# srtee/lammps-USER-CONP2

Measured on AMD Instinct MI355X. Metric: charge-solve updates/sec + ns/day, 4096-atom electrode / 32k electrolyte, higher is better.
Workload: dtype f64; 1 GPU; synthetic graphene/IL 4096 electrode + 32768 electrolyte, ffield; Ne=4096, Nl=32768, K=99773, kflat=645, mode=ffield, solver=inv, kspace=ewald, blist_pairs=302717, structure_factor_form=z-window (32 columns, grid 480)

## Files before the change

### include/conp_hip.h

```cpp
#ifndef CONP_HIP_H
#define CONP_HIP_H

#include <stddef.h>
#include <stdint.h>

#ifdef __cplusplus
extern "C" {
#endif

#define CONP_ABI_VERSION 1

typedef enum {
  CONP_OK = 0,
  CONP_ERR_ARG = -1,
  CONP_ERR_STATE = -2,
  CONP_ERR_NO_DEVICE = -3,
  CONP_ERR_NUMERIC = -4,
  CONP_ERR_IO = -5
} conp_status;

enum { CONP_FF_NORMAL = 0, CONP_FF_FFIELD = 1, CONP_FF_NOSLAB = 2 };
enum { CONP_SOLVER_CG = 0, CONP_SOLVER_INV = 1 };

typedef struct conp_fix conp_fix;
// ... 114 lines not shown
                              double *energy ,
                              double *virial ,
                              double *eatom  );

int conp_pppm_compute_forces(conp_fix *fix, const conp_atoms *atoms,
                             double *f      ,
                             double *energy ,
                             double *virial ,
                             double *eatom  );

typedef struct {
  int pairflag, kspaceflag, qsumflag;
  double eta;
} conp_potential_args;
int conp_compute_potential_atom(conp_fix *fix, const conp_atoms *atoms, const conp_neighlist *pairlist, const int *sel,
                                const int *etasel , const conp_potential_args *args, double *potential);

typedef struct {
  int elenum, elenum_all, elytenum, maxtag_all, runstage;
  int kcount, kcount_flat, kcount_expand, kxmax, kymax, kzmax, kmax, kmax3d;
  int kcount_dims[7];
  int cg_iterations;
  int n_zclasses;
  double unitk[3], volume, gsqmx, ug_tot, totsetq, scalar_output, totinve, slabcorr;
  int64_t n_blist_pairs, n_alist_pairs, n_elyte_charged;
  int inverse_path;
  int inverse_retries;
  int pppm_elyte_spreads;
  int zn_cols, zn_grid, zn_rows;
  int zn_ranges;
  int hc_arithmetic;
  int zc_final;
  int zc_row_tiles;
} conp_info;
int conp_fix_info(const conp_fix *fix, conp_info *out);
int conp_fix_get_ktables(const conp_fix *fix, int *kxvecs, int *kyvecs, int *kzvecs, double *ug, int *kxy_list, int *kz_list);
int conp_fix_get_maps(const conp_fix *fix, int *ele2tag, int *ele2eleall, int *eleall2tag, int *eleall2ele,
                      int *elecheck_eleall, int *elebuf2eleall, int *tag2eleall);
int conp_fix_get_matrix(conp_fix *fix, double *aaa_all );
int conp_fix_set_matrix(conp_fix *fix, const double *aaa_all, int runstage);
int conp_fix_get_vectors(conp_fix *fix, double *bbb_all, double *eleallq, double *elesetq);
int conp_fix_get_sfac(conp_fix *fix, double *sfacrl, double *sfacim);
int conp_fix_get_ele_trig(conp_fix *fix, double *csk, double *snk);
int conp_inv_project(conp_fix *fix, int n, double *aaa, int nullneutral, int zneutr, const double *eleallz, double zhalf,
                     double *totinve_out);

int conp_fix_write_matrix_file(conp_fix *fix, const char *path, int which);
int conp_fix_read_matrix_file(conp_fix *fix, const conp_atoms *atoms, const char *path);

int conp_invert(conp_fix *fix, int n, double *aaa);

int conp_host_ktables(double g_ewald, double accuracy, double slab_volfactor, int slabflag, double xprd, double yprd, double zprd,
                      double qsqsum, int64_t natoms, double qqrd2e, double dielectric, int *info , int *kxvecs,
                      int *kyvecs, int *kzvecs, double *ug, int *kxy_list, int *kz_list, int *plan_p, int *plan_m, int *plan_sign);
int conp_host_index(int n0, const int *tag0, const int *echeck0, int n1, const int *tag1, const int *echeck1, int *sizes,
                    int *ele2tag, int *ele2eleall, int *eleall2tag, int *eleall2ele, int *elebuf2eleall, int *tag2eleall);
int64_t conp_host_pair_rows(int which, const conp_neighlist *list, const conp_atoms *atoms, int newton, int *row_ptr,
                            int *ele_atom, int *oth_atom, int *col);

int conp_fix_set_stream(conp_fix *fix, void *hip_stream);
int conp_fix_bind_device_buffers(conp_fix *fix, double *d_b , double *d_q );
int conp_fix_row_range(const conp_fix *fix, int *row0, int *row1);
int conp_fix_b_cal_device(conp_fix *fix, const double *d_x, const double *d_q);
int conp_fix_solve_device(conp_fix *fix, double potdiff);
int conp_fix_scatter_device(conp_fix *fix, double *d_q_atoms, double potdiff);
int conp_fix_pre_force_device(conp_fix *fix, const double *d_x, double *d_q, double potdiff);
// ... 35 lines not shown
  int nlocal, nall;
  double cutneigh;
  const int *d_tag, *d_nspecial, *d_special;
  int maxspecial;
  double prd_half[3];
} conp_pair_build_args;
int conp_pair_build_list_device(conp_fix *fix, const double *d_x, const conp_pair_build_args *a);
int conp_pair_list_moved_device(conp_fix *fix, const double *d_x, double trigger, int *d_flag);
int conp_pair_get_list(conp_fix *fix, int *inum, int *nall, int64_t *nneigh,
                       int *ilist, int *numneigh, int *first, int *neigh);

int conp_fix_profile(conp_fix *fix, int enable);
int conp_fix_profile_read(conp_fix *fix, int *nkernels, const char **names , double *avg_ms , int *counts );
int conp_fix_pin_host_arrays(conp_fix *fix, const double *x, const double *q, int n);
int conp_fix_unpin_host_arrays(conp_fix *fix);
void *conp_host_alloc(size_t bytes);
void conp_host_free(void *p);

int conp_debug_check_guards(void);

enum {
  CONP_PATH_PARTIAL_TILES = 1 << 0,
  CONP_PATH_A_GENERAL = 1 << 1,
  CONP_PATH_INV_PIVOTED = 1 << 2,
  CONP_PATH_CG_TWO_LAUNCH = 1 << 3,
  CONP_PATH_GEMV_ROWS = 1 << 4,
  CONP_PATH_PHASE_LAUNCH = 1 << 5,
  CONP_PATH_PPPM_SPREAD_LAUNCH = 1 << 6,
  CONP_PATH_ROWS_HOST = 1 << 7,
  CONP_PATH_TIME_SPLIT = 1 << 8,
  CONP_PATH_SK_CLASSIC = 1 << 12,
  CONP_PATH_ZN_WIDE = 1 << 13,
  CONP_PATH_ZC_PHASE_LOADS = 1 << 14,
  CONP_PATH_HC_TABLES = 1 << 15
};
void conp_debug_set_paths(unsigned mask);
void conp_debug_set_sk_workgroups(int n);
void conp_debug_set_ew_block(int n);


int conp_fix_write_timing(conp_fix *fix);
const char *conp_fix_log_drain(conp_fix *fix);
const char *conp_fix_mesg_drain(conp_fix *fix);

#ifdef __cplusplus
}
#endif
#endif
```

### lammps-user-conp2_amd/conp_amd/capi.py

```python
from __future__ import annotations

import ctypes as C
import os
from typing import Optional, Sequence

import numpy as np

from . import systems as _systems

HERE = os.path.dirname(os.path.abspath(__file__))
_LIB = None


class ConpError(RuntimeError):
    def __init__(self, code, msg):
        super().__init__(f"[conp status {code}] {msg}")
        self.code = code
        self.msg = msg


def library_path():
    return os.environ.get("CONP_LIB") or os.path.join(HERE, "libconp_hip.so")


# ... 32 lines not shown
_CB_GATHERV = C.CFUNCTYPE(C.c_int, C.c_void_p, C.c_void_p, C.c_int64, C.c_void_p, C.POINTER(C.c_int64), C.POINTER(C.c_int64))


class conp_comm(C.Structure):
    _fields_ = [("ctx", C.c_void_p), ("rank", C.c_int), ("nranks", C.c_int), ("allreduce_sum", _CB_SUM),
                ("allreduce_max_int", _CB_MAXI), ("allgather_int", _CB_GATHER_INT), ("allgatherv", _CB_GATHERV)]


class conp_potential_args(C.Structure):
    _fields_ = [("pairflag", C.c_int), ("kspaceflag", C.c_int), ("qsumflag", C.c_int), ("eta", C.c_double)]


class conp_pair_params(C.Structure):
    _fields_ = [("ntypes", C.c_int), ("cutsq", C.POINTER(C.c_double)), ("cut_coul", C.c_double),
                ("cut_ljsq", C.POINTER(C.c_double)), ("lj1", C.POINTER(C.c_double)), ("lj2", C.POINTER(C.c_double)),
                ("lj3", C.POINTER(C.c_double)), ("lj4", C.POINTER(C.c_double)), ("offset", C.POINTER(C.c_double)),
                ("special_lj", C.c_double * 4), ("special_coul", C.c_double * 4)]


class conp_pair_build_args(C.Structure):
    _fields_ = [("nlocal", C.c_int), ("nall", C.c_int), ("cutneigh", C.c_double), ("d_tag", C.c_void_p), ("d_nspecial", C.c_void_p),
                ("d_special", C.c_void_p), ("maxspecial", C.c_int), ("prd_half", C.c_double * 3)]


class conp_info(C.Structure):
    _fields_ = [("elenum", C.c_int), ("elenum_all", C.c_int), ("elytenum", C.c_int), ("maxtag_all", C.c_int),
                ("runstage", C.c_int), ("kcount", C.c_int), ("kcount_flat", C.c_int), ("kcount_expand", C.c_int),
                ("kxmax", C.c_int), ("kymax", C.c_int), ("kzmax", C.c_int), ("kmax", C.c_int), ("kmax3d", C.c_int),
                ("kcount_dims", C.c_int * 7), ("cg_iterations", C.c_int), ("n_zclasses", C.c_int), ("unitk", C.c_double * 3),
                ("volume", C.c_double), ("gsqmx", C.c_double), ("ug_tot", C.c_double), ("totsetq", C.c_double),
                ("scalar_output", C.c_double), ("totinve", C.c_double), ("slabcorr", C.c_double),
                ("n_blist_pairs", C.c_int64), ("n_alist_pairs", C.c_int64), ("n_elyte_charged", C.c_int64),
                ("inverse_path", C.c_int), ("inverse_retries", C.c_int), ("pppm_elyte_spreads", C.c_int), ("zn_cols", C.c_int), ("zn_grid", C.c_int), ("zn_rows", C.c_int),
                ("zn_ranges", C.c_int), ("hc_arithmetic", C.c_int), ("zc_final", C.c_int), ("zc_row_tiles", C.c_int)]


SYMBOLS = [
    "conp_parse_fix_args", "conp_fix_create", "conp_fix_destroy", "conp_last_error", "conp_abi_version",
    "conp_fix_init_list", "conp_fix_setup_post_neighbor", "conp_fix_setup_pre_force", "conp_fix_post_neighbor",
    "conp_fix_pre_force", "conp_fix_compute_scalar", "conp_fix_post_force", "conp_fix_post_force_step", "conp_fix_modify_param", "conp_fix_linalg_setup", "conp_fix_a_cal", "conp_fix_b_cal",
    "conp_fix_equation_solve", "conp_fix_update_charge", "conp_km_conp_setup", "conp_km_a_cal", "conp_km_b_cal",
    "conp_fix_info", "conp_fix_get_ktables", "conp_fix_get_maps", "conp_fix_get_matrix", "conp_fix_set_matrix",
    "conp_fix_get_vectors", "conp_fix_get_sfac", "conp_fix_get_ele_trig", "conp_inv_project", "conp_invert",
    "conp_host_ktables", "conp_host_index", "conp_host_pair_rows", "conp_fix_write_matrix_file", "conp_fix_read_matrix_file",
    "conp_fix_set_stream",
    "conp_fix_bind_device_buffers", "conp_fix_row_range", "conp_fix_b_cal_device", "conp_fix_solve_device",
    "conp_fix_scatter_device", "conp_fix_pre_force_device", "conp_fix_profile", "conp_fix_profile_read", "conp_debug_check_guards",
    "conp_debug_set_paths", "conp_debug_set_sk_workgroups", "conp_debug_set_ew_block",
    "conp_fix_pin_host_arrays", "conp_fix_unpin_host_arrays", "conp_host_alloc", "conp_host_free",
    "conp_fix_write_timing", "conp_fix_log_drain", "conp_fix_mesg_drain",
    "conp_fix_set_comm", "conp_rccl_unique_id", "conp_fix_comm_init_rccl", "conp_rccl_available", "conp_fix_comm_destroy_rccl",
    "conp_pppm_make_rho", "conp_pppm_compute_group_potential", "conp_pppm_compute_particle_potential",
    "conp_pppm_keep_density", "conp_pppm_compute",
    "conp_ewald_compute", "conp_ewald_compute_group_potential", "conp_ewald_compute_particle_potential",
    "conp_ewald_compute_forces", "conp_pppm_compute_forces",
    "conp_ewald_compute_forces_device", "conp_pppm_compute_forces_device",
    "conp_ewald_compute_forces_vatom", "conp_pppm_compute_forces_vatom",
    "conp_ewald_compute_forces_vatom_device", "conp_pppm_compute_forces_vatom_device",
    "conp_compute_potential_atom",
    "conp_pair_set_params", "conp_pair_set_list", "conp_pair_compute", "conp_pair_compute_device",
    "conp_pair_build_list_device", "conp_pair_list_moved_device", "conp_pair_get_list",
]


PATH_PARTIAL_TILES, PATH_A_GENERAL, PATH_INV_PIVOTED, PATH_CG_TWO_LAUNCH, PATH_GEMV_ROWS = 1, 2, 4, 8, 16
PATH_PHASE_LAUNCH, PATH_PPPM_SPREAD_LAUNCH, PATH_ROWS_HOST, PATH_TIME_SPLIT = 32, 64, 128, 256
PATH_SK_CLASSIC = 4096
PATH_ZN_WIDE = 8192
PATH_ZC_PHASE_LOADS = 16384
PATH_HC_TABLES = 32768


class test_paths:

    def __init__(self, mask=0, sk_workgroups=0):
        self.mask, self.nwg = mask, sk_workgroups

    def __enter__(self):
        lib = load_library()
        if not hasattr(lib, "conp_debug_set_paths"):
            raise RuntimeError("this library build has no test hooks (a comparison build of an earlier round?)")
        lib.conp_debug_set_paths(self.mask)
        lib.conp_debug_set_sk_workgroups(self.nwg)
        return self

    def __exit__(self, *a):
        lib = load_library()
        lib.conp_debug_set_paths(0)
        lib.conp_debug_set_sk_workgroups(0)
        return False


def set_ew_block(n: int):
    load_library().conp_debug_set_ew_block(int(n))


def load_library():
    global _LIB
    if _LIB is not None:
        return _LIB
    path = library_path()
    if not os.path.exists(path):
        raise ImportError(f"{path} is missing: build it with `python -c 'import __graft_entry__ as g; g.build()'` "
# ... 672 lines not shown
```

### lammps-user-conp2_amd/csrc/conp_fix.cpp

```cpp
#include <hip/hip_runtime.h>
#include <dlfcn.h>
#include <rccl/rccl.h>

#include <algorithm>
#include <cmath>
#include <cstdarg>
#include <chrono>
#include <cstdio>
#include <cstdlib>
#include <cstring>
#include <map>
#include <memory>
#include <mutex>
#include <stdexcept>
#include <string>
#include <vector>

#include "../../include/conp_hip.h"
#include "conp_host.hpp"
#include "conp_kernels.h"

namespace {

thread_local std::string g_last_error;
// ... 278 lines not shown
  double cond_vmult = 0.0;
  bool cond_ready = false;
  std::vector<int> elyte_idx_h;
  int bl_inum = 0;
  size_t bl_nneigh = 0;
  DevBuf<char> d_rows_scratch;
  int nlocal_cur = 0;
  hipStream_t stream = nullptr;
  bool own_stream = false;
  DevBuf<double> d_x, d_q, d_qc, d_slab_part, d_Gpart, d_G, d_Gw, d_wfull, d_Rp, d_Tz, d_ele_z, d_bk, d_breal, d_b_own,
      d_eleallq_own, d_qele, d_elesetq, d_eleinitq, d_A, d_cutsq, d_scalars, d_ainve, d_sfr, d_sfi, d_cg_res, d_cg_p, d_Srows, d_xg, d_qg, d_pp_ele, d_pp_scratch,
      d_cg_ap, d_cg_scal, d_inv_work, d_inv_backup, d_Tzc, d_TzcT, d_Hpart, d_Hc, d_Wz, d_Spk, d_yp, d_f, d_pfacc, d_pp_coeff, d_pp_green, d_pp_tw0, d_pp_tw1,
      d_pp_tw2, d_pp_re, d_pp_im, d_pp_ew, d_eta_ij, d_fo_ij, d_u0_i, d_diag_atom, d_setzvec;
  DevBuf<double2> d_Xt, d_Yt, d_Zt, d_Xe, d_Ye;
  DevBuf<int> d_type, d_atom2eleall, d_elyte_idx, d_p_ikx, d_p_iky, d_p_sgn, d_sf_row_a, d_sf_col_c, d_k_sign, d_k_p, d_k_m,
      d_elecheck, d_zclass, d_nb_act, d_rt_mine, d_own_rt, d_own_pv, d_ele_pairs, d_a_chunk_group, d_ct_ptr, d_seg_ptr, d_seg_idx, d_hslot_ptr, d_hslot_idx, d_b_rowptr, d_b_ele, d_b_oth, d_a_rowptr, d_a_ele, d_a_oth, d_a_col, d_bl_ilist, d_bl_numneigh, d_bl_first, d_bl_neigh, d_pp_egrid, d_ipiv, d_info, d_cg_done, d_iota, d_ele_csr_ptr, d_ele_csr_of, d_ele_csr_row;
  bool left_stale = false;
  double left_potdiff = 0.0;
  DevBuf<unsigned char> d_mask;
  DevBuf<SkItem> d_items;
  DevBuf<SkWItem> d_witems;
  int witems_maxseg = 1;
  DevBuf<SkProj> d_skproj;
  SkProj skproj_h{};
  DevBuf<SkFuse> d_skfuse;
  SkFuse skfuse_h{};
  DevBuf<SkTile> d_tiles;
  double *d_b = nullptr, *d_eleallq = nullptr;
  bool b_bound = false, q_bound = false;
  int n_slab_part = 0;
  const bool sk_partials = path_on(CONP_PATH_PARTIAL_TILES);
  const bool time_split = path_on(CONP_PATH_TIME_SPLIT);
  const bool gemv_rows = path_on(CONP_PATH_GEMV_ROWS);
  const bool no_phase_fuse = path_on(CONP_PATH_PHASE_LAUNCH);
  int table_c0 = 0, table_c1 = 0;
  int hslots = 0;
  bool g_current = true;
  int max_nsplit = 0;
  int n_slots = 0;
  DevPlan dplan{};
  Profiler prof;

  ~conp_fix() {
    if (time_host && th[5] > 0)
      std::fprintf(stderr, "conp host-buffer update, us per call over %.0f calls: list check %.1f, staging + H2D enqueue %.1f, kernel "
                           "enqueue %.1f, solve enqueue + wait + D2H %.1f, scatter %.1f\n", th[5], 1e6 * th[0] / th[5], 1e6 * th[1] / th[5],
                   1e6 * th[2] / th[5], 1e6 * th[3] / th[5], 1e6 * th[4] / th[5]);
    prof.collect();
    drop_graph();
    if (nccl) { (void)hipStreamSynchronize(stream); (void)g_rccl.CommDestroy(nccl); nccl = nullptr; }
    if (pin_x || pin_q) { (void)hipStreamSynchronize(stream); if (pin_x) (void)hipHostUnregister(const_cast<double *>(pin_x)); if (pin_q) (void)hipHostUnregister(const_cast<double *>(pin_q)); }
    if (h_pin) { (void)hipStreamSynchronize(stream); (void)hipHostFree(h_pin); }
    if (h_np) { (void)hipStreamSynchronize(stream); (void)hipHostFree(h_np); }
    if (ren_arena) { (void)hipStreamSynchronize(stream); (void)hipHostFree(ren_arena); ren_arena = nullptr; }
    if (zn_flag_host) { (void)hipStreamSynchronize(stream); (void)hipHostFree(zn_flag_host); zn_flag_host = nullptr; }
    for (auto &e : ev_b) if (e) (void)hipEventDestroy(e);
    if (own_stream && stream) (void)hipStreamDestroy(stream);
  }

  RealParams real_params() const {
    RealParams rp;
    rp.g_ewald = env.g_ewald; rp.eta = args.eta;
    double cut_coulsq = env.cut_coul * env.cut_coul;
    const double cut_erfc = 5.8 * 5.8 / (env.g_ewald * env.g_ewald);
    if (cut_coulsq > cut_erfc) cut_coulsq = cut_erfc;
    rp.cut_coulsq = cut_coulsq; rp.ntypes = env.ntypes; rp.cutsq = d_cutsq.p;
// ... 1680 lines not shown
                                           "two collectives yourself between conp_fix_b_cal_device / _solve_device / _scatter_device)");
    prof.end(stream);
  }
  void allgather_q() {
    if ((env.nranks <= 1 && !nccl) || args.minimizer != CONP_SOLVER_INV) return;
    const int ne = idx.elenum_all;
    prof.begin("allgather_q", stream);
    if (nccl) {
      double *mine = d_eleallq + (size_t)env.rank * rows_per;
      g_rccl.ok(g_rccl.AllGather(mine, d_eleallq, (size_t)rows_per, ncclDouble, nccl, stream), "all-gather(q)");
    } else if (rc.active()) {
      double *h = pinned((size_t)ne_pad + 8 + (size_t)ne + rows_per) + ne_pad + 8;
      const int nr = row1 - row0;
      if (nr) HIP_TRY(hipMemcpyAsync(h + ne, d_eleallq + row0, nr * sizeof(double), hipMemcpyDeviceToHost, stream));
      sync();
      std::vector<int> rows(env.nranks);
      for (int r = 0; r < env.nranks; ++r) rows[r] = std::min(ne, (r + 1) * rows_per) - std::min(ne, r * rows_per);
      rc.gatherv(h + ne, rows, 1, h);
      HIP_TRY(hipMemcpyAsync(d_eleallq, h, ne * sizeof(double), hipMemcpyHostToDevice, stream));
    }
    prof.end(stream);
  }

  bool can_fuse_solve() const {
    return args.minimizer == CONP_SOLVER_INV && !args.conq && !args.cond && env.nranks == 1 && !nccl && !s_sharded &&
           runstage >= 3;
  }
  long s_generation = 0, spk_of = -1;
  bool spk_symmetric = false;
  DevBuf<unsigned long long> d_symstat;
  bool use_sym_gemv() const {
    return !gemv_rows && idx.elenum_all >= 2048;
  }
  void solve_scatter_fused(double *d_q_atoms, double potdiff) {
    const int ne = idx.elenum_all;
    if (use_sym_gemv()) {
      if (spk_of != s_generation) {
        d_Spk.reserve(sym_packed_doubles(ne_pad));
        d_yp.reserve((size_t)(ne_pad / 128) * ne_pad);
        d_symstat.reserve(2);
        launch_sym_pack(stream, ne, ne_pad, d_A.p, d_Spk.p, d_symstat.p);
        unsigned long long st[2] = {0, 0};
        HIP_TRY(hipMemcpyAsync(st, d_symstat.p, sizeof st, hipMemcpyDeviceToHost, stream));
        sync();
        double mx, md;
        std::memcpy(&mx, &st[0], sizeof mx); std::memcpy(&md, &st[1], sizeof md);
        spk_symmetric = md <= 1e-10 * mx;
        spk_of = s_generation;
        if (!spk_symmetric)
          mesgf("conp/hip: the solve matrix is not symmetric (max |S_ij - S_ji| = %.3g, max |S_ij| = %.3g): full rows are multiplied\n", md, mx);
      }
    }
    if (use_sym_gemv() && spk_symmetric) {
      prof.begin("gemv_charge", stream);
      launch_sym_gemv_finish(stream, ne, ne_pad, d_Spk.p, d_b, d_yp.p, d_eleallq, d_elesetq.p, args.qinit ? d_eleinitq.p : nullptr,
                             potdiff, d_ele_csr_ptr.p, d_ele_csr_of.p, d_ele_csr_row.p, d_qele.p, d_q_atoms);
      prof.end(stream);
      left_stale = true; left_potdiff = potdiff;
      HIP_TRY(hipGetLastError());
      return;
    }
    prof.begin("gemv_charge", stream);
    launch_gemv_finish(stream, ne, d_A.p, d_b, d_eleallq, d_elesetq.p, args.qinit ? d_eleinitq.p : nullptr, potdiff, d_ele_csr_ptr.p,
                       d_ele_csr_of.p, d_qele.p, d_q_atoms);
    prof.end(stream);
    left_stale = true; left_potdiff = potdiff;
    HIP_TRY(hipGetLastError());
  }

  void scatter_device(double *d_q_atoms, double potdiff, bool labelled = true) {
    const int ne = idx.elenum_all;
    if (labelled) prof.begin("charge_write", stream);
    if (args.cond) {
      if (!cond_ready) {
        std::vector<double> sq(ne), sz(ne);
        HIP_TRY(hipMemcpyAsync(sq.data(), d_elesetq.p, ne * sizeof(double), hipMemcpyDeviceToHost, stream));
        HIP_TRY(hipMemcpyAsync(sz.data(), d_setzvec.p, ne * sizeof(double), hipMemcpyDeviceToHost, stream));
        sync();
        double zOAz = 0.;
        for (int i = 0; i < ne; ++i) zOAz += sq[i] * sz[i];
        double vm = 4 * 3.14159265358979323846 * zOAz * env.zprd / (evscale * env.xprd * env.yprd);
        vm /= 1 + vm;
        vm /= zOAz;
        cond_vmult = vm;
        cond_ready = true;
      }
      launch_cond_potdiff(stream, ne, d_setzvec.p, d_eleallq, d_slab_part.p, n_slab_part, env.zprd, potdiff, cond_vmult,
                          d_scalars.p + 3);
      launch_charge_finish(stream, ne, n_ele_atoms, d_ele_pairs.p, d_elecheck.p, d_eleallq, d_elesetq.p,
                           args.qinit ? d_eleinitq.p : nullptr, 0.0, d_scalars.p + 3, d_qele.p, d_q_atoms, nullptr);
    } else if (args.conq) {
      launch_left_sum(stream, ne, d_elecheck.p, d_eleallq, d_scalars.p + 1);
      launch_conq_potdiff(stream, d_scalars.p + 1, potdiff, totsetq, env.one_electrode, d_scalars.p + 3);
      launch_charge_finish(stream, ne, n_ele_atoms, d_ele_pairs.p, d_elecheck.p, d_eleallq, d_elesetq.p,
// ... 676 lines not shown
  if (!f->tables_current) f->km_a_read(at);
  if (at->nlocal + at->nghost != f->nall) throw ConpError(CONP_ERR_STATE, "atom count changed without post_neighbor");
  if (f->elyte_list_stale(at)) { f->sync(); f->build_elyte_list(at); }
  f->upload_xq(at);
  if (f->decomposed) f->gather_elyte(at);
  f->b_cal_device(f->d_x.p, f->d_q.p, false);
  if (f->nccl || f->rc.active()) f->allreduce_b();
  HIP_TRY(hipMemcpyAsync(bbb, f->d_b, f->idx.elenum_all * sizeof(double), hipMemcpyDeviceToHost, f->stream));
  f->sync();
  CONP_GUARD_END
}

int conp_fix_info(const conp_fix *f, conp_info *o) {
  CONP_GUARD_BEGIN
  std::memset(o, 0, sizeof(*o));
  o->elenum = f->idx.elenum; o->elenum_all = f->idx.elenum_all; o->elytenum = f->idx.elytenum;
  o->maxtag_all = f->idx.maxtag_all; o->runstage = f->runstage;
  o->kcount = f->kt.kcount; o->kcount_flat = f->kt.kcount_flat; o->kcount_expand = f->kt.kcount_expand;
  o->kxmax = f->kt.kxmax; o->kymax = f->kt.kymax; o->kzmax = f->kt.kzmax; o->kmax = f->kt.kmax; o->kmax3d = f->kt.kmax3d;
  for (int i = 0; i < 7; ++i) o->kcount_dims[i] = f->kt.kcount_dims[i];
  o->cg_iterations = f->cg_iterations;
  o->n_zclasses = f->nzc;
  for (int i = 0; i < 3; ++i) o->unitk[i] = f->kt.unitk[i];
  o->volume = f->kt.volume; o->gsqmx = f->kt.gsqmx; o->ug_tot = f->kt.ug_tot; o->totsetq = f->totsetq;
  o->scalar_output = f->scalar_output; o->totinve = f->totinve; o->slabcorr = f->slabcorr;
  int64_t nbp = f->n_b_pairs;
  if (f->np_pending) { HIP_TRY(hipStreamSynchronize(f->stream)); nbp = *f->h_np; }
  o->n_blist_pairs = nbp;
  o->inverse_path = f->inverse_path; o->inverse_retries = f->inverse_retries; o->pppm_elyte_spreads = f->pp_elyte_spreads;
  const bool zn_on = f->zn_use() || f->zn_gen_use();
  o->zn_cols = zn_on ? 16 * f->zn_ncf : 0; o->zn_grid = zn_on ? f->zn_n : 0; o->zn_rows = zn_on ? 128 * (int)f->own_rt_h.size() : 0; o->n_alist_pairs = f->arows.npairs(); o->n_elyte_charged = f->nl;
  o->zn_ranges = zn_on ? f->zn_nrg : 0; o->hc_arithmetic = f->zn_use() && f->zn_frag_arith ? 1 : 0;
  o->zc_final = f->zc_final_form; o->zc_row_tiles = f->zc_final_form ? (int)f->own_rt_h.size() : 0;
  CONP_GUARD_END
}

int conp_fix_get_ktables(const conp_fix *f, int *kx, int *ky, int *kz, double *ug, int *kxy_list, int *kz_list) {
  CONP_GUARD_BEGIN
  if (!f->kspace_ready) throw ConpError(CONP_ERR_STATE, "k tables not built");
  const size_t K = f->kt.kcount, E = f->kt.kcount_expand;
  if (kx) std::memcpy(kx, f->kt.kxvecs.data(), K * sizeof(int));
  if (ky) std::memcpy(ky, f->kt.kyvecs.data(), K * sizeof(int));
  if (kz) std::memcpy(kz, f->kt.kzvecs.data(), K * sizeof(int));
  if (ug) std::memcpy(ug, f->kt.ug.data(), K * sizeof(double));
  if (kxy_list) std::memcpy(kxy_list, f->kt.kxy_list.data(), E * sizeof(int));
  if (kz_list) std::memcpy(kz_list, f->kt.kz_list.data(), E * sizeof(int));
  CONP_GUARD_END
}

int conp_fix_get_maps(const conp_fix *f, int *ele2tag, int *ele2eleall, int *eleall2tag, int *eleall2ele,
                      int *elecheck_eleall, int *elebuf2eleall, int *tag2eleall) {
  CONP_GUARD_BEGIN
  const EleIndex &x = f->idx;
  auto cp = [](int *dst, const std::vector<int> &v) { if (dst && !v.empty()) std::memcpy(dst, v.data(), v.size() * sizeof(int)); };
  cp(ele2tag, x.ele2tag); cp(ele2eleall, x.ele2eleall); cp(eleall2tag, x.eleall2tag); cp(eleall2ele, x.eleall2ele);
  cp(elecheck_eleall, x.elecheck_eleall); cp(elebuf2eleall, x.elebuf2eleall); cp(tag2eleall, x.tag2eleall);
  CONP_GUARD_END
}

int conp_fix_get_matrix(conp_fix *f, double *aaa) {
  CONP_GUARD_BEGIN
  f->drop_graph();
  f->unshard_rows();
  const size_t ne = f->idx.elenum_all;
  HIP_TRY(hipMemcpyAsync(aaa, f->d_A.p, ne * ne * sizeof(double), hipMemcpyDeviceToHost, f->stream));
  f->sync();
// ... 1216 lines not shown
```

### lammps-user-conp2_amd/csrc/conp_kernels.h

```cpp
#pragma once
#include <hip/hip_runtime.h>
#include <atomic>
#include <cstddef>
#include <cstdint>
#include "../../include/conp_hip.h"

namespace conp {

bool path_on(unsigned bit);
int debug_sk_workgroups();
int debug_ew_block();
const char *env_knob(const char *name);

struct DynLdsCache { std::atomic<size_t> granted[64]; };
template <typename K>
void ensure_dyn_lds(K kernel, size_t bytes, DynLdsCache &cache) {
  int dev = 0;
  (void)hipGetDevice(&dev);
  std::atomic<size_t> &g = cache.granted[dev & 63];
  if (bytes <= g.load(std::memory_order_relaxed)) return;
  if (hipFuncSetAttribute(reinterpret_cast<const void *>(kernel), hipFuncAttributeMaxDynamicSharedMemorySize, (int)bytes) == hipSuccess)
    g.store(bytes, std::memory_order_relaxed);
}

// ... 184 lines not shown
int sk_hc_max_classes();
void launch_project_zclass_pieces(hipStream_t s, const DevPlan &pl, int ne_pad, int n_own, const int *own_rt, int nzc, const double *Hp,
                                  const int *slot_ptr, const int *slot_idx, bool presum , const int *frag_ptr , const int2 *frag_ents , int nfrag, const double *Rp, const double2 *Xe,
                                  const double2 *Ye, const int *own_pv, const int *zclass, double *Hc, double *bk_part, const BRowArgs *fin,
                                  const BRowArgs *pairs = nullptr ,
                                  double *breal_out = nullptr,
                                  bool wide = false ,
                                  int arith_nrg = 0 ,
                                  int arith_stride = 0);
bool hc_frag_lists_arithmetic(const int *frag_ptr, const int2 *ents, int nfrag, int nrg, int stride);
size_t zc_final_phase_lds(int n_own, int nzc, int kxmax, int kymax);
void launch_sk_reduce(hipStream_t s, const DevPlan &pl, const SkTile *tiles, int ntiles, int max_nsplit, double *part, double *G,
                      double *Gwf);
void launch_sfac_gather(hipStream_t s, int kcount, int C_pad, int PT, const int *sf_row_a, const int *sf_col_c,
                        const int *k_sign, const double *G, double *sfacrl, double *sfacim);
void launch_b_project(hipStream_t s, const DevPlan &pl, int ne_pad, const int *ct_ptr , const SkTile *tiles,
                      const double *Gwf, const double *Rp, const double *Tz, double *bk_part );
void launch_reduce_project_zclass(hipStream_t s, const DevPlan &pl, const SkTile *tiles, int ntiles, int max_nsplit, double *part,
                                  double *G, int ne_pad, int n_own, const int *own_rt, int nzc, const double *Tzc, const double *Rp,
                                  const double2 *Xe , const double2 *Ye ,
                                  const int *own_pv , const int *zclass, double *Hc, double *bk_part,
                                  const BRowArgs *fin );
void launch_b_project_zclass(hipStream_t s, const DevPlan &pl, int ne_pad, const int *rt_mine, int n_own, const int *own_rt, int nzc, const double *Gwf,
                             const double *Tzc , const double *Rp, const double2 *Xe, const double2 *Ye,
                             const int *own_pv, const int *zclass ,
                             double *Hc , double *bk_part , const BRowArgs *fin);
void launch_b_real_combine(hipStream_t s, int ne, int ne_pad, int row0, int row1, const int *row_ptr, const int *ele_atom,
                           const int *oth_atom, const double *x, const double *q, const int *type, RealParams rp, int add_k,
                           const double *bk, int slab, const double *ele_z, const double *slab_part, int n_slab_part,
                           double slab_pref, double *b_out, double *slab_out,
                           const double *breal = nullptr );
size_t sym_packed_doubles(int ne_pad);
void launch_sym_pack(hipStream_t s, int ne, int ne_pad, const double *S, double *Spk, unsigned long long *stat);
void launch_sym_gemv_finish(hipStream_t s, int n, int ne_pad, const double *Spk, const double *b, double *yp ,
                            double *y, const double *elesetq, const double *eleinitq, double potdiff, const int *atoms_ptr,
                            const int *atoms_of, const int *atoms_row , double *q_ele, double *q_atoms);
void launch_gemv_rows(hipStream_t s, int n, int row0, int row1, const double *S, const double *b, double *y);
void launch_gemv_finish(hipStream_t s, int n, const double *S, const double *b, double *y, const double *elesetq,
                        const double *eleinitq, double potdiff, const int *atoms_ptr, const int *atoms_of, double *q_ele,
                        double *q_atoms);
void launch_charge_finish(hipStream_t s, int ne, int nall, const int *atom2eleall, const int *elecheck, const double *eleallq,
                          const double *elesetq, const double *eleinitq, double potdiff, const double *d_potdiff, double *q_ele,
                          double *q_atoms, double *left_out);
void launch_cond_potdiff(hipStream_t s, int ne, const double *setzvec, const double *eleallq, const double *slab_part,
                         int n_slab_part, double lz, double rightcharge, double vmult, double *out);
void launch_conq_potdiff(hipStream_t s, const double *left, double rightcharge, double totsetq, int one_electrode, double *out);
size_t b_rows_scratch_bytes(int ne, size_t nneigh);
void launch_atom2eleall(hipStream_t s, int nall, int npairs, const int *pairs , int *atom2eleall );
void launch_build_b_rows(hipStream_t s, int inum, size_t nneigh, const int *ilist, const int *numneigh, const int *first,
                         const int *neigh, const int *arow, int nlocal, int newton, int ne, void *scratch, size_t scratch_bytes,
                         int *row_ptr, int *ele, int *oth, unsigned *np_pinned );
void launch_post_force(hipStream_t s, int inum, const int *ilist, const int *numneigh, const int *first, const int *neigh, int nlocal,
                       int nall, int newton, const double *x,
                       const double *q, const int *type, const int *atom2eleall, RealParams rp, double qqrd2e, double *f,
                       double *acc , bool clear_f);
constexpr int PAIR_TAB_W = 8;
constexpr int PAIR_LDS_ENTRIES = 256;
struct PairArgs {
  int inum;
  const int *ilist, *numneigh, *first, *neigh;
  int nlocal, newton;
  const double4 *xq;
  const int *type;
  int nt1, ntab;
  const double *tab;
  double cut_coulsq, g_ewald, qqrd2e;
  double special_lj[4], special_coul[4];
// ... 65 lines not shown
```

### lammps-user-conp2_amd/csrc/conp_kernels.hip

```cpp
#include "conp_kernels.h"
#include "conp_brow.hpp"

#include <atomic>
#include <cstdio>
#include <cstdlib>

namespace conp {

typedef double d4 __attribute__((ext_vector_type(4)));
#define MFMA_F64(a, b, c) __builtin_amdgcn_mfma_f64_16x16x4f64((a), (b), (c), 0, 0, 0)

const char *env_knob(const char *name) {
  const char *v = getenv(name);
  if (v) {
    static std::atomic<unsigned long long> said{0};
    unsigned h = 0;
    for (const char *c = name; *c; ++c) h = h * 31u + (unsigned char)*c;
    const unsigned long long bit = 1ull << (h & 63u);
    if (!(said.fetch_or(bit) & bit))
      fprintf(stderr, "libconp_hip: %s=%s is set -- a non-default code path is in use\n", name, v);
  }
  return v;
}
static std::atomic<unsigned> g_paths{0};
// ... 1520 lines not shown
#pragma unroll
  for (int i = 0; i < 8; ++i) {
    const bool hi = lane & 32;
    const double keep = hi ? p[8 + i] : p[i], send = hi ? p[i] : p[8 + i];
    p[i] = keep + __shfl_xor(send, 32, 64);
  }
#pragma unroll
  for (int i = 0; i < 4; ++i) {
    const bool hi = lane & 16;
    const double keep = hi ? p[4 + i] : p[i], send = hi ? p[i] : p[4 + i];
    p[i] = keep + __shfl_xor(send, 16, 64);
  }
#pragma unroll
  for (int i = 0; i < 2; ++i) {
    const bool hi = lane & 8;
    const double keep = hi ? p[2 + i] : p[i], send = hi ? p[i] : p[2 + i];
    p[i] = keep + __shfl_xor(send, 8, 64);
  }
  {
    const bool hi = lane & 4;
    const double keep = hi ? p[1] : p[0], send = hi ? p[0] : p[1];
    p[0] = keep + __shfl_xor(send, 4, 64);
  }
  p[0] += __shfl_xor(p[0], 2, 64);
  return p[0] + __shfl_xor(p[0], 1, 64);
}

#ifdef SYM_TIMELINE
__device__ unsigned long long sym_tl[4096 * 3];
#define SYM_STAMP(k) do { if (threadIdx.x == 0 && blockIdx.x < 4096) sym_tl[blockIdx.x * 3 + (k)] = wall_clock64(); } while (0)
#else
#define SYM_STAMP(k) do { } while (0)
#endif
__global__ __launch_bounds__(256, 4) void sym_gemv_kernel(int ne, int ne_pad, const double *__restrict__ Spk, const double *__restrict__ b,
                                                          double *__restrict__ yp ) {
  __shared__ double bi_s[SG_T], bj_s[SG_T];
  __shared__ double tr[4][SG_T];
  SYM_STAMP(0);
  int t = blockIdx.x, bi = 0;
  while ((bi + 1) * (bi + 2) / 2 <= t) ++bi;
  const int bj = t - bi * (bi + 1) / 2;
  const unsigned tid = threadIdx.x, lane = tid & 63, wave = tid >> 6;
  const double2 *tile = reinterpret_cast<const double2 *>(Spk + (size_t)t * SG_T * SG_T) + (size_t)(32 * wave) * 64 + lane;
  double2 v[16];
#pragma unroll
  for (int r = 0; r < 16; ++r) v[r] = tile[r * 64];
  {
    const int i = (tid < SG_T ? bi : bj) * SG_T + (int)(tid & (SG_T - 1));
    (tid < SG_T ? bi_s : bj_s)[tid & (SG_T - 1)] = i < ne ? b[i] : 0.0;
  }
  __syncthreads();
  const double bj0 = bj_s[2 * lane], bj1 = bj_s[2 * lane + 1];
  double at0 = 0.0, at1 = 0.0;
  double *ydir = yp + (size_t)bj * ne_pad + bi * SG_T + 32 * wave + (lane >> 2);
#pragma unroll
  for (int h = 0; h < 2; ++h) {
    double p[16];
#pragma unroll
    for (int r = 0; r < 16; ++r) {
      p[r] = fma(v[r].y, bj1, v[r].x * bj0);
      const double br = bi_s[32 * wave + 16 * h + r];
      at0 = fma(v[r].x, br, at0);
      at1 = fma(v[r].y, br, at1);
    }
    if (h == 0) {
      unsigned off2 = 16 * 64;
      asm volatile("" : "+v"(off2) : "v"(at0), "v"(at1));
#pragma unroll
      for (int r = 0; r < 16; ++r) v[r] = tile[off2 + r * 64];
    }
    const double rs = wave_sum16_transposed(p, lane);
    if ((lane & 3) == 0) ydir[16 * h] = rs;
  }
  if (bi != bj) {
    tr[wave][2 * lane] = at0; tr[wave][2 * lane + 1] = at1;
    __syncthreads();
    if (tid < SG_T) yp[(size_t)bi * ne_pad + bj * SG_T + tid] = (tr[0][tid] + tr[1][tid]) + (tr[2][tid] + tr[3][tid]);
  }
#ifdef SYM_TIMELINE
  __syncthreads();
  SYM_STAMP(1);
  if (threadIdx.x == 0 && blockIdx.x < 4096) {
    unsigned hw, xcc;
    asm volatile("s_getreg_b32 %0, hwreg(HW_REG_HW_ID)" : "=s"(hw));
    asm volatile("s_getreg_b32 %0, hwreg(HW_REG_XCC_ID)" : "=s"(xcc));
    sym_tl[blockIdx.x * 3 + 2] = ((unsigned long long)xcc << 32) | hw;
  }
#endif
}

constexpr int SF_R = 32;
__global__ __launch_bounds__(4 * SF_R) void sym_finish_kernel(int n, int ne_pad, int nb, const double *__restrict__ yp, double *__restrict__ y,
                                                         const double *__restrict__ elesetq, const double *__restrict__ eleinitq,
                                                         double potdiff, const int *__restrict__ atoms_ptr,
                                                         const int *__restrict__ atoms_of, const int *__restrict__ atoms_row,
                                                         double *__restrict__ q_ele, double *__restrict__ q_atoms) {
  __shared__ double part[4][SF_R];
  __shared__ double vq[SF_R];
  const int rl = threadIdx.x & (SF_R - 1), g = threadIdx.x / SF_R;
  const int row0 = blockIdx.x * SF_R, row = row0 + rl;
  const int rend = row0 + SF_R < n ? row0 + SF_R : n;
  int k0 = 0, k1 = 0;
  if (q_atoms) { k0 = atoms_ptr[row0]; k1 = atoms_ptr[rend]; }
  double sq = 0.0, iq = 0.0;
  if (g == 0 && row < n) { sq = elesetq[row]; if (eleinitq) iq = eleinitq[row]; }
  double s = 0.0;
  if (row < n) {
    for (int kb = g; kb < nb; kb += 32) {
      double w[8];
#pragma unroll
      for (int u = 0; u < 8; ++u) w[u] = kb + 4 * u < nb ? yp[(size_t)(kb + 4 * u) * ne_pad + row] : 0.0;
#pragma unroll
      for (int u = 0; u < 8; ++u) s += w[u];
    }
  }
  part[g][rl] = s;
  __syncthreads();
  if (g == 0 && row < n) {
    const double r = (part[0][rl] + part[1][rl]) + (part[2][rl] + part[3][rl]);
    double v;
    {
#pragma clang fp contract(off)
      v = r + potdiff * sq;
      if (eleinitq) v += iq;
    }
    y[row] = r; q_ele[row] = v;
    vq[rl] = v;
  }
  __syncthreads();
  if (!q_atoms) return;
  for (int k = k0 + (int)threadIdx.x; k < k1; k += 4 * SF_R) q_atoms[atoms_of[k]] = vq[atoms_row[k] - row0];
}

#ifdef SYM_TIMELINE
extern "C" int conp_debug_sym_timeline(unsigned long long *out, int nblocks) {
  return (int)hipMemcpyFromSymbol(out, HIP_SYMBOL(sym_tl), sizeof(unsigned long long) * 3 * (size_t)nblocks);
}
#endif
size_t sym_packed_doubles(int ne_pad) { const size_t nb = ne_pad / SG_T; return nb * (nb + 1) / 2 * SG_T * SG_T; }
void launch_sym_pack(hipStream_t s, int ne, int ne_pad, const double *S, double *Spk, unsigned long long *stat) {
  const int nb = ne_pad / SG_T;
  (void)hipMemsetAsync(stat, 0, 2 * sizeof(unsigned long long), s);
  hipLaunchKernelGGL(sym_pack_kernel, dim3(nb * (nb + 1) / 2), dim3(256), 0, s, ne, S, Spk, stat);
}
void launch_sym_gemv_finish(hipStream_t s, int n, int ne_pad, const double *Spk, const double *b, double *yp, double *y,
                            const double *elesetq, const double *eleinitq, double potdiff, const int *atoms_ptr, const int *atoms_of,
                            const int *atoms_row, double *q_ele, double *q_atoms) {
  const int nb = ne_pad / SG_T;
  hipLaunchKernelGGL(sym_gemv_kernel, dim3(nb * (nb + 1) / 2), dim3(256), 0, s, n, ne_pad, Spk, b, yp);
  hipLaunchKernelGGL(sym_finish_kernel, dim3((n + SF_R - 1) / SF_R), dim3(4 * SF_R), 0, s, n, ne_pad, nb, (const double *)yp, y, elesetq, eleinitq,
                     potdiff, atoms_ptr, atoms_of, atoms_row, q_ele, q_atoms);
}

void launch_gemv_rows(hipStream_t s, int n, int row0, int row1, const double *S, const double *b, double *y) {
  if (row1 <= row0) return;
  if (gemv_nt((size_t)(row1 - row0) * n * sizeof(double)))
    hipLaunchKernelGGL(gemv_rows_kernel<true>, dim3((row1 - row0 + 3) / 4), dim3(256), 0, s, n, row0, row1, S, b, y);
  else
    hipLaunchKernelGGL(gemv_rows_kernel<false>, dim3((row1 - row0 + 3) / 4), dim3(256), 0, s, n, row0, row1, S, b, y);
}

__global__ __launch_bounds__(256) void charge_finish_kernel(int ne, int nall, const int *__restrict__ atom2eleall,
                                                            const int *__restrict__ elecheck, const double *__restrict__ eleallq,
                                                            const double *__restrict__ elesetq, const double *__restrict__ eleinitq,
                                                            double potdiff, const double *__restrict__ d_potdiff,
                                                            double *__restrict__ q_ele,
                                                            double *__restrict__ q_atoms, double *__restrict__ left_out) {
#pragma clang fp contract(off)
  if (d_potdiff) potdiff = *d_potdiff;
  if (blockIdx.x == gridDim.x - 1) {
    if (!left_out) return;
    __shared__ double red[4];
    double s16[16];
#pragma unroll
    for (int u = 0; u < 16; ++u) s16[u] = 0.0;
    for (int i0 = threadIdx.x; i0 < ne; i0 += 4096) {
      int ec[16];
      double v[16];
#pragma unroll
      for (int u = 0; u < 16; ++u) {
        const int i = i0 + 256 * u;
        ec[u] = i < ne ? elecheck[i] : 0;
        v[u] = i < ne ? eleallq[i] : 0.0;
      }
// ... 759 lines not shown
```

Baseline: 12080 updates/s.

## Split symmetric packed GEMV tiles across two half-tile workgroups by default

The symmetric packed-matrix GEMV used for the inverse charge solve now splits each 128x128 triangular tile between two 128-thread workgroups by default. Each workgroup handles half the tile rows. The transposed contributions from the two halves go to separate slot buffers, and the finish kernel sums them. The aim is more workgroups in flight and better latency hiding on the 4096-row packed matrix, which otherwise launches few blocks. The cost is extra partial-sum storage, extra reads in the finish kernel, and redundant loads of the b vector. A debug path flag keeps the old whole-tile path.

```diff
diff --git a/include/conp_hip.h b/include/conp_hip.h
--- a/include/conp_hip.h
+++ b/include/conp_hip.h
@@ -170,6 +170,7 @@
   int hc_arithmetic;
   int zc_final;
   int zc_row_tiles;
+  int sym_units;
 } conp_info;
 int conp_fix_info(const conp_fix *fix, conp_info *out);
 int conp_fix_get_ktables(const conp_fix *fix, int *kxvecs, int *kyvecs, int *kzvecs, double *ug, int *kxy_list, int *kz_list);
@@ -271,7 +272,8 @@
   CONP_PATH_SK_CLASSIC = 1 << 12,
   CONP_PATH_ZN_WIDE = 1 << 13,
   CONP_PATH_ZC_PHASE_LOADS = 1 << 14,
-  CONP_PATH_HC_TABLES = 1 << 15
+  CONP_PATH_HC_TABLES = 1 << 15,
+  CONP_PATH_SYM_WHOLE_TILES = 1 << 16
 };
 void conp_debug_set_paths(unsigned mask);
 void conp_debug_set_sk_workgroups(int n);
diff --git a/lammps-user-conp2_amd/conp_amd/capi.py b/lammps-user-conp2_amd/conp_amd/capi.py
--- a/lammps-user-conp2_amd/conp_amd/capi.py
+++ b/lammps-user-conp2_amd/conp_amd/capi.py
@@ -88,7 +88,8 @@
                 ("scalar_output", C.c_double), ("totinve", C.c_double), ("slabcorr", C.c_double),
                 ("n_blist_pairs", C.c_int64), ("n_alist_pairs", C.c_int64), ("n_elyte_charged", C.c_int64),
                 ("inverse_path", C.c_int), ("inverse_retries", C.c_int), ("pppm_elyte_spreads", C.c_int), ("zn_cols", C.c_int), ("zn_grid", C.c_int), ("zn_rows", C.c_int),
-                ("zn_ranges", C.c_int), ("hc_arithmetic", C.c_int), ("zc_final", C.c_int), ("zc_row_tiles", C.c_int)]
+                ("zn_ranges", C.c_int), ("hc_arithmetic", C.c_int), ("zc_final", C.c_int), ("zc_row_tiles", C.c_int),
+                ("sym_units", C.c_int)]
 
 
 SYMBOLS = [
@@ -125,6 +126,7 @@
 PATH_ZN_WIDE = 8192
 PATH_ZC_PHASE_LOADS = 16384
 PATH_HC_TABLES = 32768
+PATH_SYM_WHOLE_TILES = 65536
 
 
 class test_paths:
diff --git a/lammps-user-conp2_amd/csrc/conp_fix.cpp b/lammps-user-conp2_amd/csrc/conp_fix.cpp
--- a/lammps-user-conp2_amd/csrc/conp_fix.cpp
+++ b/lammps-user-conp2_amd/csrc/conp_fix.cpp
@@ -334,6 +334,7 @@
   const bool sk_partials = path_on(CONP_PATH_PARTIAL_TILES);
   const bool time_split = path_on(CONP_PATH_TIME_SPLIT);
   const bool gemv_rows = path_on(CONP_PATH_GEMV_ROWS);
+  const bool sym_whole = path_on(CONP_PATH_SYM_WHOLE_TILES);
   const bool no_phase_fuse = path_on(CONP_PATH_PHASE_LAUNCH);
   int table_c0 = 0, table_c1 = 0;
   int hslots = 0;
@@ -2080,12 +2081,14 @@
   bool use_sym_gemv() const {
     return !gemv_rows && idx.elenum_all >= 2048;
   }
+  int sym_units() const { return sym_whole ? 1 : 2; }
+  int sym_units_ran = 0;
   void solve_scatter_fused(double *d_q_atoms, double potdiff) {
     const int ne = idx.elenum_all;
     if (use_sym_gemv()) {
       if (spk_of != s_generation) {
         d_Spk.reserve(sym_packed_doubles(ne_pad));
-        d_yp.reserve((size_t)(ne_pad / 128) * ne_pad);
+        d_yp.reserve(sym_slot_doubles(ne_pad, sym_units()));
         d_symstat.reserve(2);
         launch_sym_pack(stream, ne, ne_pad, d_A.p, d_Spk.p, d_symstat.p);
         unsigned long long st[2] = {0, 0};
@@ -2101,13 +2104,14 @@
     }
     if (use_sym_gemv() && spk_symmetric) {
       prof.begin("gemv_charge", stream);
-      launch_sym_gemv_finish(stream, ne, ne_pad, d_Spk.p, d_b, d_yp.p, d_eleallq, d_elesetq.p, args.qinit ? d_eleinitq.p : nullptr,
+      launch_sym_gemv_finish(stream, sym_units_ran = sym_units(), ne, ne_pad, d_Spk.p, d_b, d_yp.p, d_eleallq, d_elesetq.p, args.qinit ? d_eleinitq.p : nullptr,
                              potdiff, d_ele_csr_ptr.p, d_ele_csr_of.p, d_ele_csr_row.p, d_qele.p, d_q_atoms);
       prof.end(stream);
       left_stale = true; left_potdiff = potdiff;
       HIP_TRY(hipGetLastError());
       return;
     }
+    sym_units_ran = 0;
     prof.begin("gemv_charge", stream);
     launch_gemv_finish(stream, ne, d_A.p, d_b, d_eleallq, d_elesetq.p, args.qinit ? d_eleinitq.p : nullptr, potdiff, d_ele_csr_ptr.p,
                        d_ele_csr_of.p, d_qele.p, d_q_atoms);
@@ -2850,6 +2854,7 @@
   o->zn_cols = zn_on ? 16 * f->zn_ncf : 0; o->zn_grid = zn_on ? f->zn_n : 0; o->zn_rows = zn_on ? 128 * (int)f->own_rt_h.size() : 0; o->n_alist_pairs = f->arows.npairs(); o->n_elyte_charged = f->nl;
   o->zn_ranges = zn_on ? f->zn_nrg : 0; o->hc_arithmetic = f->zn_use() && f->zn_frag_arith ? 1 : 0;
   o->zc_final = f->zc_final_form; o->zc_row_tiles = f->zc_final_form ? (int)f->own_rt_h.size() : 0;
+  o->sym_units = f->sym_units_ran;
   CONP_GUARD_END
 }
 
diff --git a/lammps-user-conp2_amd/csrc/conp_kernels.h b/lammps-user-conp2_amd/csrc/conp_kernels.h
--- a/lammps-user-conp2_amd/csrc/conp_kernels.h
+++ b/lammps-user-conp2_amd/csrc/conp_kernels.h
@@ -240,7 +240,8 @@
                            const double *breal = nullptr );
 size_t sym_packed_doubles(int ne_pad);
 void launch_sym_pack(hipStream_t s, int ne, int ne_pad, const double *S, double *Spk, unsigned long long *stat);
-void launch_sym_gemv_finish(hipStream_t s, int n, int ne_pad, const double *Spk, const double *b, double *yp ,
+size_t sym_slot_doubles(int ne_pad, int units);
+void launch_sym_gemv_finish(hipStream_t s, int units, int n, int ne_pad, const double *Spk, const double *b, double *yp,
                             double *y, const double *elesetq, const double *eleinitq, double potdiff, const int *atoms_ptr,
                             const int *atoms_of, const int *atoms_row , double *q_ele, double *q_atoms);
 void launch_gemv_rows(hipStream_t s, int n, int row0, int row1, const double *S, const double *b, double *y);
diff --git a/lammps-user-conp2_amd/csrc/conp_kernels.hip b/lammps-user-conp2_amd/csrc/conp_kernels.hip
--- a/lammps-user-conp2_amd/csrc/conp_kernels.hip
+++ b/lammps-user-conp2_amd/csrc/conp_kernels.hip
@@ -1576,33 +1576,42 @@
 #else
 #define SYM_STAMP(k) do { } while (0)
 #endif
-__global__ __launch_bounds__(256, 4) void sym_gemv_kernel(int ne, int ne_pad, const double *__restrict__ Spk, const double *__restrict__ b,
-                                                          double *__restrict__ yp ) {
-  __shared__ double bi_s[SG_T], bj_s[SG_T];
-  __shared__ double tr[4][SG_T];
+template <int U>
+__global__ __launch_bounds__(256 / U, 4) void sym_gemv_kernel(int ne, int ne_pad, const double *__restrict__ Spk, const double *__restrict__ b,
+                                                              double *__restrict__ yp ,
+                                                              double *__restrict__ ypt ) {
+  constexpr int W = 4 / U;
+  constexpr int RU = SG_T / U;
+  __shared__ double bi_s[RU], bj_s[SG_T];
+  __shared__ double tr[W][SG_T];
   SYM_STAMP(0);
-  int t = blockIdx.x, bi = 0;
+  const int t = blockIdx.x / U, p = blockIdx.x % U;
+  int bi = 0;
   while ((bi + 1) * (bi + 2) / 2 <= t) ++bi;
   const int bj = t - bi * (bi + 1) / 2;
   const unsigned tid = threadIdx.x, lane = tid & 63, wave = tid >> 6;
-  const double2 *tile = reinterpret_cast<const double2 *>(Spk + (size_t)t * SG_T * SG_T) + (size_t)(32 * wave) * 64 + lane;
+  const double2 *tile = reinterpret_cast<const double2 *>(Spk + (size_t)t * SG_T * SG_T) + (size_t)(RU * p + 32 * wave) * 64 + lane;
   double2 v[16];
 #pragma unroll
   for (int r = 0; r < 16; ++r) v[r] = tile[r * 64];
-  {
+  if constexpr (U == 1) {
     const int i = (tid < SG_T ? bi : bj) * SG_T + (int)(tid & (SG_T - 1));
     (tid < SG_T ? bi_s : bj_s)[tid & (SG_T - 1)] = i < ne ? b[i] : 0.0;
+  } else {
+    const int j = bj * SG_T + (int)tid, i = bi * SG_T + RU * p + (int)tid;
+    bj_s[tid] = j < ne ? b[j] : 0.0;
+    if (tid < RU) bi_s[tid] = i < ne ? b[i] : 0.0;
   }
   __syncthreads();
   const double bj0 = bj_s[2 * lane], bj1 = bj_s[2 * lane + 1];
   double at0 = 0.0, at1 = 0.0;
-  double *ydir = yp + (size_t)bj * ne_pad + bi * SG_T + 32 * wave + (lane >> 2);
+  double *ydir = yp + (size_t)bj * ne_pad + bi * SG_T + RU * p + 32 * wave + (lane >> 2);
 #pragma unroll
   for (int h = 0; h < 2; ++h) {
-    double p[16];
+    double p16[16];
 #pragma unroll
     for (int r = 0; r < 16; ++r) {
-      p[r] = fma(v[r].y, bj1, v[r].x * bj0);
+      p16[r] = fma(v[r].y, bj1, v[r].x * bj0);
       const double br = bi_s[32 * wave + 16 * h + r];
       at0 = fma(v[r].x, br, at0);
       at1 = fma(v[r].y, br, at1);
@@ -1613,13 +1622,17 @@
 #pragma unroll
       for (int r = 0; r < 16; ++r) v[r] = tile[off2 + r * 64];
     }
-    const double rs = wave_sum16_transposed(p, lane);
+    const double rs = wave_sum16_transposed(p16, lane);
     if ((lane & 3) == 0) ydir[16 * h] = rs;
   }
   if (bi != bj) {
     tr[wave][2 * lane] = at0; tr[wave][2 * lane + 1] = at1;
     __syncthreads();
-    if (tid < SG_T) yp[(size_t)bi * ne_pad + bj * SG_T + tid] = (tr[0][tid] + tr[1][tid]) + (tr[2][tid] + tr[3][tid]);
+    if constexpr (U == 1) {
+      if (tid < SG_T) yp[(size_t)bi * ne_pad + bj * SG_T + tid] = (tr[0][tid] + tr[1][tid]) + (tr[2][tid] + tr[3][tid]);
+    } else {
+      ypt[((size_t)p * (ne_pad / SG_T) + bi) * ne_pad + bj * SG_T + tid] = tr[0][tid] + tr[1][tid];
+    }
   }
 #ifdef SYM_TIMELINE
   __syncthreads();
@@ -1634,7 +1647,10 @@
 }
 
 constexpr int SF_R = 32;
-__global__ __launch_bounds__(4 * SF_R) void sym_finish_kernel(int n, int ne_pad, int nb, const double *__restrict__ yp, double *__restrict__ y,
+static_assert(SG_T % SF_R == 0, "a finishing block lies inside one row block");
+template <int U>
+__global__ __launch_bounds__(4 * SF_R) void sym_finish_kernel(int n, int ne_pad, int nb, const double *__restrict__ yp,
+                                                         const double *__restrict__ ypt , double *__restrict__ y,
                                                          const double *__restrict__ elesetq, const double *__restrict__ eleinitq,
                                                          double potdiff, const int *__restrict__ atoms_ptr,
                                                          const int *__restrict__ atoms_of, const int *__restrict__ atoms_row,
@@ -1650,10 +1666,26 @@
   if (g == 0 && row < n) { sq = elesetq[row]; if (eleinitq) iq = eleinitq[row]; }
   double s = 0.0;
   if (row < n) {
+    [[maybe_unused]] const int R = row0 / SG_T;
     for (int kb = g; kb < nb; kb += 32) {
       double w[8];
-#pragma unroll
-      for (int u = 0; u < 8; ++u) w[u] = kb + 4 * u < nb ? yp[(size_t)(kb + 4 * u) * ne_pad + row] : 0.0;
+      if constexpr (U == 1) {
+#pragma unroll
+        for (int u = 0; u < 8; ++u) w[u] = kb + 4 * u < nb ? yp[(size_t)(kb + 4 * u) * ne_pad + row] : 0.0;
+      } else {
+        const double *ypt1 = ypt + (size_t)nb * ne_pad;
+        double w1[8];
+#pragma unroll
+        for (int u = 0; u < 8; ++u) {
+          const int sl = kb + 4 * u;
+          const bool in = sl < nb, tp = in && sl > R;
+          const double *src = tp ? ypt : yp;
+          w[u] = in ? src[(size_t)sl * ne_pad + row] : 0.0;
+          w1[u] = tp ? ypt1[(size_t)sl * ne_pad + row] : 0.0;
+        }
+#pragma unroll
+        for (int u = 0; u < 8; ++u) w[u] = kb + 4 * u > R ? w[u] + w1[u] : w[u];
+      }
 #pragma unroll
       for (int u = 0; u < 8; ++u) s += w[u];
     }
@@ -1687,13 +1719,21 @@
   (void)hipMemsetAsync(stat, 0, 2 * sizeof(unsigned long long), s);
   hipLaunchKernelGGL(sym_pack_kernel, dim3(nb * (nb + 1) / 2), dim3(256), 0, s, ne, S, Spk, stat);
 }
-void launch_sym_gemv_finish(hipStream_t s, int n, int ne_pad, const double *Spk, const double *b, double *yp, double *y,
+size_t sym_slot_doubles(int ne_pad, int units) { return (size_t)(units == 2 ? 3 : 1) * (ne_pad / SG_T) * ne_pad; }
+void launch_sym_gemv_finish(hipStream_t s, int units, int n, int ne_pad, const double *Spk, const double *b, double *yp, double *y,
                             const double *elesetq, const double *eleinitq, double potdiff, const int *atoms_ptr, const int *atoms_of,
                             const int *atoms_row, double *q_ele, double *q_atoms) {
-  const int nb = ne_pad / SG_T;
-  hipLaunchKernelGGL(sym_gemv_kernel, dim3(nb * (nb + 1) / 2), dim3(256), 0, s, n, ne_pad, Spk, b, yp);
-  hipLaunchKernelGGL(sym_finish_kernel, dim3((n + SF_R - 1) / SF_R), dim3(4 * SF_R), 0, s, n, ne_pad, nb, (const double *)yp, y, elesetq, eleinitq,
-                     potdiff, atoms_ptr, atoms_of, atoms_row, q_ele, q_atoms);
+  const int nb = ne_pad / SG_T, ntile = nb * (nb + 1) / 2;
+  double *ypt = yp + (size_t)nb * ne_pad;
+  if (units == 2) {
+    hipLaunchKernelGGL(sym_gemv_kernel<2>, dim3(2 * ntile), dim3(128), 0, s, n, ne_pad, Spk, b, yp, ypt);
+    hipLaunchKernelGGL(sym_finish_kernel<2>, dim3((n + SF_R - 1) / SF_R), dim3(4 * SF_R), 0, s, n, ne_pad, nb, (const double *)yp,
+                       (const double *)ypt, y, elesetq, eleinitq, potdiff, atoms_ptr, atoms_of, atoms_row, q_ele, q_atoms);
+  } else {
+    hipLaunchKernelGGL(sym_gemv_kernel<1>, dim3(ntile), dim3(256), 0, s, n, ne_pad, Spk, b, yp, (double *)nullptr);
+    hipLaunchKernelGGL(sym_finish_kernel<1>, dim3((n + SF_R - 1) / SF_R), dim3(4 * SF_R), 0, s, n, ne_pad, nb, (const double *)yp,
+                       (const double *)nullptr, y, elesetq, eleinitq, potdiff, atoms_ptr, atoms_of, atoms_row, q_ele, q_atoms);
+  }
 }
 
 void launch_gemv_rows(hipStream_t s, int n, int row0, int row1, const double *S, const double *b, double *y) {
```

Measured after the change: 12090 updates/s (median of 3 runs). About the same (+0.1%).
